# hidasib/GRU4Rec

Measured on AMD Instinct MI355X. Metric: mini-batches/sec (gru4rec.py:661), RSC15-shaped batch=128 n_sample=2048 BPR-max, higher is better.
Workload: dtype f32

## Files before the change

gru4rec_amd/build.py:

```python
import glob
import os
import subprocess
import sys

HERE = os.path.dirname(os.path.abspath(__file__))
SRC = os.path.join(HERE, 'csrc', 'g4r_api.hip')
SRC_HOST = os.path.join(HERE, 'csrc', 'g4r_io.cpp')
OUT = os.path.join(HERE, 'libgru4rec_hip.so')
DEPS = sorted(p for ext in ('hip', 'cuh', 'hpp', 'cpp') for p in glob.glob(os.path.join(HERE, 'csrc', '*.' + ext))) + \
       [os.path.join(os.path.dirname(HERE), 'include', 'gru4rec_hip.h'), os.path.abspath(__file__)]


def build(force=False, verbose=False, out=None, defs=(), flags=()):
    if out is not None:
        return _compile(out, list(defs), verbose, list(flags))
    if not force and os.path.exists(OUT) and all(os.path.getmtime(OUT) >= os.path.getmtime(d) for d in DEPS):
        return OUT
    return _compile(OUT, [], verbose)


COMMON_FLAGS = ['-mllvm', '-amdgpu-kernarg-preload-count=16']


MUTANTS = {1: 'sparse accumulator increments x 1.01', 2: 'sparse Adagrad steps x 1.01', 3: 'dense accumulator increments x 1.01',
# ... 7 lines not shown
           10: "k_replay_final (g4r_recommend_sessions) reads every row's final state from the buffer of the chunk's LONGEST history",
           11: "k_score_cand (g4r_score_candidates*): a work item past a row's first slice reads the items of the row's first slice",
           12: "the two-stage top-k (g4r_recommend_*_scan) ranks its candidates by the APPROXIMATE bf16 scores: the fp32 re-scoring is skipped",
           13: "cosine (g4r_similar_items): the candidate's inverse norm is read at the candidate POSITION instead of its item index",
           14: "k_rollout_feed (g4r_continue_sessions): the sorted insertion drops an item that sorts ABOVE every item already in the row's "
               "exclusion list, so it is never excluded and can be generated again",
           15: "k_beam_advance (g4r_beam_sessions) reads the hidden state of beam row i ITSELF instead of the row of its parent: a new beam "
               "carries on from the wrong state wherever the selection re-parents",
           16: "the owner walk of k_sparse_update_generic drops the first hit of every pass after the first (an item with more than 64 "
               "earlier occurrences in a step loses one of them per later pass)",
           17: "opt_rule's new second statistic (adadelta's update average, Adam's mean) x 1.01",
           18: "k_loss_rows' grp_fast takes a group of V columns whose last column is the first inactive in-batch one (column M) as wholly "
               "active: the unmasked copy of the element loops runs over it",
           19: "k_loss_rows' first pass starts its loop past the prefetched groups one STEP late: the columns of the first trip keep "
               "whatever the LDS held",
           20: "gumbel_noise (g4r_sample_sessions) ignores the decoding step (Philox counter word 2 = 0): every step of a draw gets the "
               "noise of step 0",
           21: "k_owner_window takes the sample-store row of every step of its window from the window's FIRST global step: the owner "
               "tables of the later steps are those of another list",
           22: "hidden_act_bwd decides the branch of leaky / elu / selu on the VALUE of the stored candidate (c >= 0), not on its sign bit: "
               "a pre-activation whose result rounds to -0.0 gets the positive branch's slope",
           23: "hidden_act_bwd: the negative-branch slope of leaky / elu / selu x 1.01",
           24: "k_mmr_rerank (g4r_diversify_*): from the second update on, a position's largest similarity to the picks is OVERWRITTEN by "
               "its similarity to the last pick instead of max-ed with it"}


def mutant_path(k):
    return os.path.join(HERE, '_variants', 'libgru4rec_hip_mut%d.so' % k)


def build_mutants(force=False, verbose=False):
    import fcntl
    from concurrent.futures import ThreadPoolExecutor
    os.makedirs(os.path.join(HERE, '_variants'), exist_ok=True)

    def stale():
        return [k for k in MUTANTS if force or not os.path.exists(mutant_path(k)) or
                any(os.path.getmtime(mutant_path(k)) < os.path.getmtime(d) for d in DEPS)]
    if not stale():
        return [mutant_path(k) for k in MUTANTS]
    with open(os.path.join(HERE, '_variants', '.lock'), 'w') as lock:
        fcntl.flock(lock, fcntl.LOCK_EX)
        todo = stale()
        if todo:
            _host_object(verbose)
            with ThreadPoolExecutor(min(len(todo), 2)) as ex:
                list(ex.map(lambda k: _device(mutant_path(k), ['G4R_MUTATE=%d' % k], verbose, audit=(k != 4)), todo))
# ... 108 lines not shown
```

gru4rec_amd/csrc/g4r_device.cuh:

```cuda
#pragma once
#include <hip/hip_runtime.h>
#include <stdint.h>

#include "../../include/gru4rec_hip.h"

typedef float f32x4 __attribute__((ext_vector_type(4)));

#define G4R_EPS_LOSS 1e-24f
#define G4R_EPS_ADAGRAD 1e-6f
#define G4R_OWN_INLINE 15
#define G4R_OWN_SLOTS 16
#define G4R_OWN_WINDOW_MAXR 12288
#define G4R_OWN_WINDOW_MINWG 4

#if defined(G4R_MUTATE) && G4R_MUTATE == 1
#define G4R_MUT_ACC(x) ((x) * 1.01f)
#else
#define G4R_MUT_ACC(x) (x)
#endif
#if defined(G4R_MUTATE) && G4R_MUTATE == 2
#define G4R_MUT_STEP(x) ((x) * 1.01f)
#else
#define G4R_MUT_STEP(x) (x)
#endif
#if defined(G4R_MUTATE) && G4R_MUTATE == 3
#define G4R_MUT_DACC(x) ((x) * 1.01f)
#else
#define G4R_MUT_DACC(x) (x)
#endif

#if defined(G4R_MUTATE) && G4R_MUTATE == 6
#define G4R_MUT_ROW(n, x) ((n) == 0 ? (x) * 1.5f : (x))
#else
#define G4R_MUT_ROW(n, x) (x)
// ... 13 lines not shown
#else
#define G4R_MUT_PASS_SKIP(pass, ri) false
#endif
#if defined(G4R_MUTATE) && G4R_MUTATE == 17
#define G4R_MUT_STAT2(x) ((x) * 1.01f)
#else
#define G4R_MUT_STAT2(x) (x)
#endif
#if defined(G4R_MUTATE) && G4R_MUTATE == 18
#define G4R_MUT_FAST_M(M) ((M) + 1)
#else
#define G4R_MUT_FAST_M(M) (M)
#endif
#if defined(G4R_MUTATE) && G4R_MUTATE == 19
#define G4R_MUT_FIRST_LATE(step) (step)
#else
#define G4R_MUT_FIRST_LATE(step) 0
#endif

#if defined(G4R_MUTATE) && G4R_MUTATE == 21
#define G4R_MUT_WIN_G(g0, s) (g0)
#else
#define G4R_MUT_WIN_G(g0, s) ((g0) + (s))
#endif

#define G4R_STREAM_SAMPLE 0x53414D50u
#define G4R_STREAM_DROP_EMBED 0x44454D42u
#define G4R_STREAM_DROP_HIDDEN 0x44484944u
#define G4R_STREAM_TIEBREAK 0x54494542u

#if defined(__HIP_DEVICE_COMPILE__)
#define GAS __attribute__((address_space(1)))
#else
#define GAS
#endif
#define GP(T) GAS T*

__device__ __forceinline__ float4 ld4(const GAS float* p) { return *(const GAS float4*)p; }
__device__ __forceinline__ void st4(GAS float* p, float4 v) { *(GAS float4*)p = v; }
__device__ __forceinline__ int4 ldi4(const GAS int* p) { return *(const GAS int4*)p; }
#if defined(__HIP_DEVICE_COMPILE__)
__device__ __forceinline__ float4 ld4(const float* p) { return *(const float4*)p; }
__device__ __forceinline__ void st4(float* p, float4 v) { *(float4*)p = v; }
#endif
__device__ __forceinline__ float4 ld4_if(const GAS float* base, size_t off, bool ok) {
    const float4 v = ld4(base + (ok ? off : (size_t)0));
// ... 263 lines not shown
```

gru4rec_amd/csrc/g4r_host_create.hpp:

```cpp

int g4r_device_count(void) {
    int n = 0;
    if (hipGetDeviceCount(&n) != hipSuccess) return 0;
    return n;
}
const char* g4r_last_error(void) { return g_err.c_str(); }
#ifndef G4R_HIPCC_VERSION
#define G4R_HIPCC_VERSION "unknown"
#endif
const char* g4r_version(void) { return "gru4rec_hip 0.4 (gfx950; hipcc " G4R_HIPCC_VERSION "; isa-audited)"; }
int g4r_sizeof_config(void) { return (int)sizeof(g4r_config); }

static int build_lean_args(g4r_model* m) {
    DevModel& d = m->dm;
    const StepKernels& k = m->kern;
    const int L = d.n_layers;
    std::vector<LeanV> av(L); std::vector<LeanH> ah(L); std::vector<LeanDa> aa(L); std::vector<LeanDy> ay(L);
    const bool constrained = d.embed_mode == G4R_EMBED_CONSTRAINED;
    bool any_layer = false;
    for (int l = 0; l < L; ++l) {
        if (k.fwd[l] != FWD_LEAN) continue;
        any_layer = true;
        LeanV& v = av[l]; memset(&v, 0, sizeof(v));
        v.Wx = d.dense_p + d.offWx[l]; v.Wrz = d.dense_p + d.offWrz[l]; v.Bh = d.dense_p + d.offBh[l];
// ... 33 lines not shown
        q.col_item = d.col_item; q.occ_idx = d.occ_idx + d.B; q.occ_fl = d.occ_fl; q.mp = nullptr; q.dbg = d.dbgclk; q.dbgtile = d.dbgtile; q.R = d.R; q.pub_fl = d.xmode == 0 ? 1 : 0; q.logq = d.logq;
        m->h_leanS = q;
        if (dalloc(m, &m->d_leanS, (size_t)1)) return -1;
    }
    if (k.score_bwd == SB_LEAN) {
        LeanB q; memset(&q, 0, sizeof(q));
        q.accBy = d.accBy; q.occ_fl = d.occ_fl; q.dSy = d.dSy; q.dAy = d.dAy; q.dSBy = d.dSBy; q.dABy = d.dABy; q.dhpart = d.dhpart; q.dbg = d.dbgclk; q.dbgtile = d.dbgtile;
        q.dSy_stride = d.dSy_stride; q.dSBy_stride = d.dSBy_stride; q.defer_mask = d.defer_mask; q.generic = d.generic;
        q.ndh = cdiv(d.Dtop + 1, 64); q.nA = cdiv(d.ldSc, 16) * q.ndh; q.nrb = cdiv(d.B, 16); q.ndb = cdiv(d.Dtop, 64); q.lr = d.lr;
        m->h_leanB = q;
        if (dalloc(m, &m->d_leanB, (size_t)1)) return -1;
        HIPCHK(hipMemcpyAsync(m->d_leanB, &m->h_leanB, sizeof(LeanB), hipMemcpyHostToDevice, m->stream));
    }
    if (k.update == UP_LEAN) {
        LeanU u; memset(&u, 0, sizeof(u));
        u.mp = nullptr; u.st = d.st; u.Wy = d.Wy; u.E = d.E; u.accWy = d.accWy; u.accE = d.accE; u.velWy = d.velWy; u.velE = d.velE;
        u.By = d.By; u.accBy = d.accBy; u.velBy = d.velBy; u.dAx = d.dAx; u.dAy = d.dAy; u.dABy = d.dABy;
        u.dense_p = d.dense_p; u.dense_acc = d.dense_acc; u.dense_vel = d.dense_vel; u.yin0 = d.yin0; u.meta = d.cur_in + 2 * d.B;
        u.dbg = d.dbgclk; u.dbgtile = d.dbgtile; u.n_items = d.n_items; u.constrained = constrained ? 1 : 0; u.wE = d.Ein; u.wY = d.Dtop;
        u.lr = d.lr; u.mom = d.mom; u.lmbd = d.lmbd;
        m->h_leanU = u;
        const std::vector<DenseTile> tiles = dense_tiles(d, 16, 64);
        m->ntiles16 = (int)tiles.size();
        const size_t nslot = cdiv((long long)G4R_OWN_SLOTS * d.R * 16 * sizeof(int), (long long)sizeof(DenseTile));
        if (dalloc(m, &m->d_tiles16, tiles.size() + nslot) || dalloc(m, &m->d_leanU, (size_t)1)) return -1;
        d.own_pos = m->sw.owner_scan_in_update ? nullptr : (int*)(m->d_tiles16 + tiles.size());
        m->h_leanU.own_on = d.own_pos ? 1 : 0;
        const bool pays = cdiv(d.R, LOSS_NW) > G4R_OWN_WINDOW_MINWG;
        m->own_window = d.own_pos && d.R <= G4R_OWN_WINDOW_MAXR && (m->sw.owner_window > 0 || (m->sw.owner_window < 0 && pays));
        HIPCHK(hipMemcpyAsync(m->d_tiles16, tiles.data(), tiles.size() * sizeof(DenseTile), hipMemcpyHostToDevice, m->stream));
        HIPCHK(hipStreamSynchronize(m->stream));
    }
    HIPCHK(hipStreamSynchronize(m->stream));
    return 0;
}

static KernelSwitches read_switches(const g4r_config& cfg) {
    KernelSwitches w;
    w.no_lean = getenv("G4R_NO_LEAN") != nullptr; w.no_mt = getenv("G4R_NO_MT") != nullptr; w.no_bmt = getenv("G4R_NO_BMT") != nullptr;
    w.no_merge = getenv("G4R_NO_MERGE") != nullptr; w.owner_scan_in_update = env_int("G4R_OWNER_SCAN", 0) != 0;
    w.owner_window = env_int("G4R_OWNER_WINDOW", -1);
    w.score_b_split = env_int("G4R_SCORE_B_SPLIT", 1) != 0;
    w.allow_lean_update = env_int("G4R_LEAN_UPDATE", 1) != 0; w.defer = env_int("G4R_DEFER", cfg.defer_updates) != 0;
    w.p2_geo = env_int("G4R_P2_GEO", -1); w.ba_geo = env_int("G4R_BA_GEO", -1);
    w.wide2 = env_int("G4R_WIDE2", -1); w.p1_ks = env_int("G4R_P1_KS", 128); w.bb_ks = env_int("G4R_BB_KS", 0);
    const char* skip = getenv("G4R_SKIP_KN");
    w.skip_kn = skip ? strtoull(skip, nullptr, 0) : 0ull;
    w.trace = getenv("G4R_TRACE") != nullptr;
    return w;
}

int g4r_create(const g4r_config* cfg, g4r_model** out) {
    if (!cfg || !out) return fail("null argument");
    if (cfg->n_layers < 1 || cfg->n_layers > G4R_MAX_LAYERS) return fail("n_layers out of range");
    if (cfg->batch_size < 1 || cfg->n_items < 1) return fail("batch_size / n_items must be positive");
    for (int l = 0; l < cfg->n_layers; ++l)
        if (cfg->layers[l] % 4 != 0 || cfg->layers[l] < 4 || cfg->layers[l] > 1024)
            return fail("layer sizes must be multiples of 4 in [4, 1024]");
    if (cfg->embed_mode == G4R_EMBED_SEPARATE && (cfg->embedding % 4 != 0 || cfg->embedding < 4 || cfg->embedding > 1024))
        return fail("embedding must be a multiple of 4 in [4, 1024]");
    if (cfg->embed_mode != G4R_EMBED_CONSTRAINED && cfg->embed_mode != G4R_EMBED_SEPARATE && cfg->embed_mode != G4R_EMBED_ONEHOT)
        return fail("unsupported embedding mode");
    if (cfg->embed_mode == G4R_EMBED_ONEHOT && 3 * cfg->layers[0] > 1024)
        return fail("one-hot input: 3 * layers[0] must be <= 1024 (row width of the Wx[0] table)");
// ... 225 lines not shown
```

gru4rec_amd/csrc/g4r_host_debug.hpp:

```cpp
int g4r_get_debug(g4r_model* m, const char* name, float* host, int64_t count) {
    if (!m || !name || !host) return fail("null argument");
    HIPCHK(hipSetDevice(m->cfg.device));
    DevModel& d = m->dm;
    const StepKernels& k = m->kern;
    std::string s(name);
    const float* p = nullptr; int64_t n = 0;
    int l = 0;
    if (!s.empty() && isdigit((unsigned char)s.back())) { l = s.back() - '0'; s.pop_back(); }
    if (l >= d.n_layers) return fail("layer out of range");
    const int64_t bd = (int64_t)d.B * d.D[l];
    if (s == "scores") { p = d.Sc; n = (int64_t)d.B * d.ldSc; }
    else if (s == "dSx") { p = d.dSx + (size_t)((m->gstep - 1) & d.defer_mask) * (size_t)d.dSx_stride; n = (int64_t)d.B * d.Ein; }
    else if (s == "dSy") { p = d.dSy + (size_t)((m->gstep - 1) & d.defer_mask) * (size_t)d.dSy_stride; n = (int64_t)d.ldSc * d.Dtop; }
    else if (s == "dSBy") { p = d.dSBy + (size_t)((m->gstep - 1) & d.defer_mask) * (size_t)d.dSBy_stride; n = d.ldSc; }
    else if (s == "defer_stats") {
        if (count < 4) return fail("count");
        double rows = 0, bias = 0;
        if (m->defer_on) {
            std::vector<unsigned> st(2048);
            HIPCHK(hipStreamSynchronize(m->stream));
            HIPCHK(hipMemcpy(st.data(), d.dstat, st.size() * sizeof(unsigned), hipMemcpyDeviceToHost));
            for (size_t i = 0; i < st.size(); i += 2) { rows += st[i]; bias += st[i + 1]; }
        }
        host[0] = (float)rows; host[1] = (float)bias; host[2] = m->defer_on ? 1.f : 0.f; host[3] = (float)(d.defer_mask + 1);
// ... 15 lines not shown
        host[0] = (float)m->ro_calls; host[1] = (float)m->ro_steps;
        return 0;
    }
    else if (s == "events_launches") {
        if (count < 4) return fail("count");
        host[0] = (float)m->ev_steps; host[1] = (float)m->ev_scans; host[2] = (float)m->ev_launches; host[3] = (float)m->ev_pieces;
        return 0;
    }
    else if (s == "dhpart") { p = d.dhpart; n = (int64_t)d.ksplit * d.B * d.Dtop; }
    else if (s == "lossrow") { p = d.lossrow; n = d.B; }
    else if (s == "hd") { p = d.hd[l]; n = bd; }
    else if (s == "r") { p = d.r[l]; n = bd; }
    else if (s == "z") { p = d.z[l]; n = bd; }
    else if (s == "c") { p = d.c[l]; n = bd; }
    else if (s == "Hr") { p = d.Hr[l]; n = bd; }
    else if (s == "dV") { p = d.dV[l]; n = bd * 3; }
    else if (s == "dyl") { p = d.dyl[l]; n = bd; }
    else if (s == "Hprev") { p = d.H[l][(m->gstep + 1) & 1]; n = bd; }
    else if (s == "occ_idx") { p = (const float*)d.occ_idx; n = d.R; }
    else if (s == "own_pos") {
        if (!d.own_pos) return fail("no owner table (k_update_l not chosen, or G4R_OWNER_SCAN=1)");
        p = (const float*)(d.own_pos + (m->own_window ? (size_t)m->own_last * d.R * 16 : (size_t)0)); n = 16 * (int64_t)d.R;
    }
    else if (s == "own_pos_ring") { if (!d.own_pos) return fail("no owner table (k_update_l not chosen, or G4R_OWNER_SCAN=1)"); p = (const float*)d.own_pos; n = (int64_t)G4R_OWN_SLOTS * 16 * d.R; }
    else if (s == "owner_window") { if (count < 1) return fail("count"); host[0] = (m->own_window && k.update == UP_LEAN) ? 1.f : 0.f; return 0; }
#if !defined(G4R_CLK_TRACE)
    else if (s == "dbgclk" || s == "dbgtile") return fail("in-kernel traces need a library built with G4R_BUILD_CLK=1 (python -m gru4rec_amd.build --force) and G4R_CLK=1 at run time");
#endif
    else if (s == "dbgclk") { if (!d.dbgclk) return fail("G4R_CLK not set"); p = (const float*)d.dbgclk; n = 2 * (64 + 8 * (int64_t)d.R); }
    else if (s == "dbgtile") { if (!d.dbgtile) return fail("G4R_CLK not set"); p = (const float*)d.dbgtile; n = 2 * 8 * (int64_t)8192; }
    else if (s == "ntiles") { if (count < 1) return fail("count"); host[0] = (float)m->ntiles; return 0; }
    else if (s == "ldSc") { if (count < 1) return fail("count"); host[0] = (float)d.ldSc; return 0; }
    else if (s == "wide_mask") {
        if (count < 1) return fail("count");
        int mk = k.wide_dense ? 16 : 0;
        for (int l = 0; l < d.n_layers; ++l) mk |= k.wg[l].use;
        host[0] = (float)mk; return 0;
    }
    else if (s == "deep_geo") {
        if (count < 1) return fail("count");
        host[0] = (float)(k.p2_deep[0] + 2 * k.ba_deep[0]); return 0;
    }
    else if (s == "score_mt") { if (count < 1) return fail("count"); host[0] = k.score_fwd == SF_MT ? 272.f : 0.f; return 0; }
    else if (s == "score_bmt") { if (count < 1) return fail("count"); host[0] = (float)k.bmt_slabs; return 0; }
    else if (s == "lean") {
        if (count < 4) return fail("count");
        int mk = 0;
// ... 208 lines not shown
```

gru4rec_amd/csrc/g4r_host_model.hpp:

```cpp
static thread_local std::string g_err;
static int fail(const std::string& s) { g_err = s; return -1; }
void g4r_set_error(const char* fmt, ...) {
    char buf[1024];
    va_list ap;
    va_start(ap, fmt);
    vsnprintf(buf, sizeof(buf), fmt, ap);
    va_end(ap);
    g_err = buf;
}
#define HIPCHK(x)                                                                                        \
    do {                                                                                                 \
        hipError_t e_ = (x);                                                                             \
        if (e_ != hipSuccess)                                                                            \
            return fail(std::string(#x) + ": " + hipGetErrorString(e_) + " @" + std::to_string(__LINE__)); \
    } while (0)
#define NCCLCHK(x)                                                                                         \
    do {                                                                                                   \
        ncclResult_t e_ = (x);                                                                             \
        if (e_ != ncclSuccess)                                                                             \
            return fail(std::string(#x) + ": " + ncclGetErrorString(e_) + " @" + std::to_string(__LINE__)); \
    } while (0)

enum { KN_GRU_P1 = 0, KN_GRU_P2, KN_SCORE_FWD, KN_LOSS, KN_SCORE_BWD, KN_BWD_PRE, KN_BWD_A, KN_BWD_B, KN_DENSE, KN_ALLREDUCE,
       KN_DENSE_APPLY, KN_SPARSE, KN_UPDATE, KN_BWD_FUSED, KN_FWD_FUSED, KN_GATE, KN_FLUSH, KN_SCAN, KN_FINISH, KN_GRU_V, KN_GRU_H, KN_GRU_DA, KN_GRU_DY, KN_OWNER_WINDOW, KN_COUNT };
static const char* KN_NAMES[KN_COUNT] = {"k_gru_p1", "k_gru_p2", "k_score_fwd", "k_loss_rows", "k_score_bwd", "k_gru_bwd_pre",
                                         "k_gru_bwd_a", "k_gru_bwd_b", "k_dense_grad", "rccl_allreduce", "k_dense_apply",
                                         "k_sparse_update", "k_update", "k_gru_bwd", "k_gru_fwd", "k_gru_gate", "k_sparse_flush", "k_defer_scan", "k_finish_rows", "k_gru_v", "k_gru_h", "k_gru_da", "k_gru_dy", "k_owner_window"};

struct EvRec { int kn; hipEvent_t a, b; };

struct KernelSwitches {
    bool no_lean = false;
    bool no_mt = false, no_bmt = false;
    bool no_merge = false;
    bool allow_lean_update = true;
    bool score_b_split = true;
    bool owner_scan_in_update = false;
    int owner_window = -1;
    bool defer = false;
    int p2_geo = -1, ba_geo = -1;
    int wide2 = -1, p1_ks = 128, bb_ks = 0;
    unsigned long long skip_kn = 0;
    bool trace = false;
};
enum GruFwdKind { FWD_LEAN = 0 , FWD_FUSED = 1 , FWD_P1S = 2 ,
                  FWD_P1_N64 = 3, FWD_P1_N32 = 4 };
enum GruBwdKind { BWD_LEAN = 0 , BWD_FUSED = 1 , BWD_ONEHOT = 2, BWD_BW = 3, BWD_B = 4 };
enum ScoreFwdKind { SF_LEAN = 0 , SF_MT = 1 , SF_T3 = 2, SF_T2 = 3, SF_K64 = 4, SF_K128 = 5  };
enum ScoreBwdKind { SB_LEAN = 0 , SB_BMT = 1 , SB_BWD2 = 2 , SB_W = 3, SB_N = 4  };
enum UpdateKind { UP_LEAN = 0 , UP_MERGED = 1 , UP_SPLIT = 2 };
struct WideGeo { int use = 0, ny = 1, nh = 1, kys = 0, khs = 0, bbn = 1, bbk = 0; };
struct StepKernels {
    int fwd[G4R_MAX_LAYERS], bwd[G4R_MAX_LAYERS];
    int p2_deep[G4R_MAX_LAYERS], ba_deep[G4R_MAX_LAYERS];
    WideGeo wg[G4R_MAX_LAYERS];
    int score_fwd;
    int loss_spec, loss_long, loss_quads;
    int score_bwd;
    int score_a_host;
    int kch, ksplit;
    int bmt_slabs;
// ... 33 lines not shown
    int64_t gstep = 0;
    DenseTile* d_tiles = nullptr;
    int ntiles = 0, nblk_occ = 0, nblk_occ_g = 0;
    size_t smem_score = 0, smem_loss = 0, smem_sparse = 0;
    bool defer_on = false;
    bool defer_broken = false;
    hipEvent_t ev_df[4] = {nullptr, nullptr, nullptr, nullptr};
    DenseTile* d_tiles64 = nullptr;
    int ntiles64 = 0;
    float* d_tmpH = nullptr;
    LeanS h_leanS;
    std::vector<LeanV> h_leanV; std::vector<LeanH> h_leanH; std::vector<LeanDa> h_leanDa; std::vector<LeanDy> h_leanDy;
    LeanS* d_leanS = nullptr;
    LeanB* d_leanB = nullptr; LeanB h_leanB;
    LeanU* d_leanU = nullptr; LeanU h_leanU;
    DenseTile* d_tiles16 = nullptr; int ntiles16 = 0;
    bool own_window = false;
    int own_last = 0;
    hipEvent_t ev_ow[2] = {nullptr, nullptr};
    LeanV* d_leanV = nullptr; LeanH* d_leanH = nullptr; LeanDa* d_leanDa = nullptr; LeanDy* d_leanDy = nullptr;
    hipGraphExec_t gexec = nullptr;
    hipGraphExec_t gexec_small = nullptr;
    hipGraphExec_t gexec_head = nullptr;
    int graph_steps = 0;
    bool dist_graph_failed = false;
    bool profiling = false;
    bool profile_split = false;
    bool exact = false;
    size_t smem_exact = 0;
    double kn_ms[KN_COUNT] = {0};
    int64_t kn_n[KN_COUNT] = {0};
    std::vector<hipEvent_t> evs;
    int pbatch = 0, ppar = 0;
    float* pH[G4R_MAX_LAYERS][2] = {{nullptr}};
    float* phout[G4R_MAX_LAYERS] = {nullptr};
    float *pVc[G4R_MAX_LAYERS] = {nullptr}, *pz[G4R_MAX_LAYERS] = {nullptr}, *pHr[G4R_MAX_LAYERS] = {nullptr};
    int *p_in = nullptr, *p_tgt = nullptr, *p_keep = nullptr;
    DevBuf<int> p_items;
    unsigned char* p_zero = nullptr;
    float* p_ranks = nullptr;
    DevBuf<float> p_scores;
    int* p_cnt = nullptr;
    int64_t p_nsel = 0, p_ldo = 0;
    DevBuf<uint2> p_topk;
    DevBuf<int> p_tcols;
    DevBuf<float> p_tscores;
    DevBuf<long long> p_xoffs;
// ... 51 lines not shown
    std::vector<SyncPlane> planes[2];
    int sync_rule[2] = {G4R_SYNC_MEAN, G4R_SYNC_SUM};
    bool sync_rule_user = false;
    unsigned char* d_touched = nullptr;
    unsigned char* d_rowcnt = nullptr;
    int sync_every_dev = 0;
    int64_t since_sync = 0, n_dev_syncs = 0;
    struct Scratch { void* p = nullptr; size_t cap = 0; bool host = false; };
    Scratch sc_ids, sc_blk, sc_cnt, sc_all, sc_send, sc_pack, sc_recv, sc_hall;
    float* d_dense[2] = {nullptr, nullptr};
    bool sync_on = false;
};

struct MmrStage {
    int tab; const float* T; int W;
    bool cosine;
    float lam; int normalize;
    int k;
    int32_t* out_pos; float* out_value;
};

static inline void weights_changed(g4r_model* m) { m->s_tab_valid = false; m->sim_valid[0] = m->sim_valid[1] = false; }
static inline void drop_step_graphs(g4r_model* m, bool also_head) {
    for (hipGraphExec_t* g : {&m->gexec, &m->gexec_small, also_head ? &m->gexec_head : nullptr})
        if (g && *g) { (void)hipGraphExecDestroy(*g); *g = nullptr; }
}

enum StepMode { STEP_GRAPH, STEP_HEAD_GRAPH, STEP_EAGER };
static inline bool local_staged(const g4r_model* m) {
    return !m->dm.apply_dense_inplace && m->cfg.nranks <= 1 && !m->comm_ready && !m->p2p_ready && !m->virtual_ranks;
}
static inline bool dist_graph_wanted(const g4r_model* m) {
    return !m->dm.apply_dense_inplace && !m->dist_graph_failed && (m->p2p_ready || m->comm_ready || local_staged(m));
}
static inline StepMode step_mode(const g4r_model* m) {
    if (!m->cfg.use_graph || m->profiling || m->sw.trace) return STEP_EAGER;
    return (m->dm.apply_dense_inplace || dist_graph_wanted(m)) ? STEP_GRAPH : STEP_HEAD_GRAPH;
}
static inline StepMode single_step_mode(const g4r_model* m, StepMode mode) {
    if (mode != STEP_GRAPH) return mode;
    return m->dm.apply_dense_inplace ? STEP_EAGER : STEP_HEAD_GRAPH;
}

template <class T>
static int dalloc(g4r_model* m, T** p, size_t n, bool zero = true) {
    void* q = nullptr;
    if (n == 0) n = 1;
    HIPCHK(hipMalloc(&q, n * sizeof(T)));
// ... 61 lines not shown
static const size_t SMEM_P1 = tile_smem<GT_BM, GT_BN, P1_BK, false, false>() + GT_BM * sizeof(int);
static constexpr auto k_gru_p2_w4 = k_gru_p2<GT_NTH, GT_BK>;
static constexpr auto k_gru_p2_w8d = k_gru_p2<512, 256>;
static const size_t SMEM_P2_256 = tile_smem<GT_BM, GT_BN, 256, false, false>() + GT_BM * sizeof(int);
static constexpr auto k_gru_bwd_a_w4 = k_gru_bwd_a<GT_NTH, GT_BK>;
static constexpr auto k_gru_bwd_a_w8d = k_gru_bwd_a<512, 256>;
static const size_t SMEM_BA_256 = tile_smem<GT_BM, GT_BN, 256, false, true>();
static const size_t SMEM_BB = tile_smem<GT_BM, GT_BN, BB_BK, false, true>() + GT_BM * sizeof(int);
static constexpr auto k_score_fwd_k128 = k_score_fwd<GT_BN, GT_BK>;
#define SFW_BN 32
#define SFW_BK 64
static constexpr auto k_score_fwd_k64 = k_score_fwd<SFW_BN, SFW_BK>;
static constexpr auto k_score_fwd_t2 = k_score_fwd<64, 32, T2_BK>;
static const size_t SMEM_SF2 = (size_t)Tile2Cfg<T2_BK>::SMEM_FLOATS * sizeof(float);
static constexpr auto k_score_fwd_t3 = k_score_fwd<64, 32, 3>;
static const size_t SMEM_SF3 = (size_t)Tile3Cfg<T3_NST, T3_BKS>::SMEM_FLOATS * sizeof(float);
static const size_t SMEM_BMT = std::max((size_t)BMT_NST_A * BMT_STAGE_A * sizeof(float), (size_t)BMT_NST_B * BMT_STAGE_B * sizeof(float) + 2048 * sizeof(int));
static const size_t SMEM_SF64 = tile_smem<SF_BM, SFW_BN, SFW_BK, false, true>() + SFW_BN * sizeof(int);
static constexpr auto k_score_bwd_n = k_score_bwd<32, GT_BK>;
static constexpr auto k_score_bwd_w = k_score_bwd<64, 64>;
static const size_t SMEM_SBW = std::max(tile_smem<64, 64, 64, true, false>(), tile_smem<64, 64, 64, false, false>());
#define ZROW_FLOATS 8192
#define G4R_DEFER_SLOTS 16
static_assert(G4R_OWN_SLOTS == G4R_DEFER_SLOTS, "the windows of g4r_train_steps serve the deferral ring and the owner ring alike");
static const size_t SMEM_SF = tile_smem<SF_BM, GT_BN, GT_BK, false, true>() + GT_BN * sizeof(int);
static constexpr auto k_score_mt_4s = k_score_mt<4, true>;
static const size_t SMEM_MT_4S = (size_t)MtCfg<4, true>::SMEM_FLOATS * sizeof(float);
static const size_t SMEM_T2K = (size_t)(4 * 64 * 16) * sizeof(float);
static const size_t SMEM_T3 = (size_t)Tile3Cfg<3, 32>::SMEM_FLOATS * sizeof(float);

static constexpr decltype(&k_loss_rows<false, 0, 1>) K_LOSS_ROWS[3][4] = {
    {k_loss_rows<false, 0, 1>, k_loss_rows<false, 1, 1>, k_loss_rows<false, 2, 1>, k_loss_rows<false, 3, 1>},
    {k_loss_rows<false, 0, 4>, k_loss_rows<false, 1, 4>, k_loss_rows<false, 2, 4>, k_loss_rows<false, 3, 4>},
    {k_loss_rows<true, 0, 4>, k_loss_rows<true, 1, 4>, k_loss_rows<true, 2, 4>, k_loss_rows<true, 3, 4>}};
static inline auto loss_rows_kernel(const StepKernels& k) { return K_LOSS_ROWS[k.loss_long ? 2 : (k.loss_quads ? 1 : 0)][k.loss_spec]; }
static inline int chunk_index(int chunks) { return chunks == 1 ? 0 : (chunks == 2 ? 1 : 2); }
static constexpr decltype(&k_sparse_update<1, false>) K_SPARSE_UPDATE[3][2] = {
    {k_sparse_update<1, false>, k_sparse_update<1, true>}, {k_sparse_update<2, false>, k_sparse_update<2, true>}, {k_sparse_update<4, false>, k_sparse_update<4, true>}};
static constexpr decltype(&k_sparse_update_generic<1>) K_SPARSE_UPDATE_GENERIC[3] = {k_sparse_update_generic<1>, k_sparse_update_generic<2>, k_sparse_update_generic<4>};
static constexpr decltype(&k_update<1, 32, false>) K_UPDATE[2][2] = {{k_update<1, 32, false>, k_update<1, 32, true>}, {k_update<2, 32, false>, k_update<2, 32, true>}};

static std::vector<DenseTile> dense_tiles(const DevModel& d, int TR, int TC) {
    std::vector<DenseTile> tiles;
    for (int l = 0; l < d.n_layers; ++l) {
        const int D = d.D[l], IN = d.IN[l];
        auto add = [&](const float* x0, const float* x1, int ldx, int nrows, int ncols, int coff, int ldo, long long base) {
            for (int r = 0; r < nrows; r += TR)
// ... 115 lines not shown
```

gru4rec_amd/csrc/g4r_host_step.hpp:

```cpp
extern "C++" {
struct StepLauncher {
    g4r_model* m;
    hipStream_t s;
    std::vector<EvRec>* recs;
    size_t evi = 0;
    int kn = -1;
    hipEvent_t ev_a = nullptr, ev_b = nullptr;
    StepLauncher(g4r_model* m_, std::vector<EvRec>* recs_) : m(m_), s(m_->stream), recs(recs_) {}
    void use(int kn_, hipEvent_t a, hipEvent_t b) { kn = kn_; ev_a = a; ev_b = b; }
    void open(int kn_) {
        if (m->sw.trace) { fprintf(stderr, "[g4r] launch %s\n", KN_NAMES[kn_]); fflush(stderr); }
        use(kn_, nullptr, nullptr);
        if (!recs) return;
        while (m->evs.size() < evi + 2) { hipEvent_t e; (void)hipEventCreate(&e); m->evs.push_back(e); }
        use(kn_, m->evs[evi], m->evs[evi + 1]);
        evi += 2;
        recs->push_back(EvRec{kn_, ev_a, ev_b});
    }
    bool skipped() const { return m->sw.skip_kn && kn >= 0 && ((m->sw.skip_kn >> kn) & 1ull); }
    template <class... P, class... A>
    void launch(void (*kern)(P...), dim3 grid, dim3 block, size_t smem, A... a) {
        if (skipped()) return;
        if (ev_a) hipExtLaunchKernelGGL(kern, grid, block, (unsigned)smem, s, ev_a, ev_b, 0, static_cast<P>(a)...);
        else hipLaunchKernelGGL(kern, grid, block, smem, s, static_cast<P>(a)...);
// ... 312 lines not shown
    e = hipGraphInstantiate(out, graph, nullptr, nullptr, 0);
    (void)hipGraphDestroy(graph);
    if (e != hipSuccess) { *out = nullptr; (void)hipGetLastError(); return fail(std::string("graph instantiate: ") + hipGetErrorString(e)); }
    return 0;
}
static int ensure_graph(g4r_model* m) {
    if (m->gexec) return 0;
    const bool dist = !m->dm.apply_dense_inplace && !local_staged(m);
    const bool rccl_in_graph = dist && (!m->p2p_ready || (m->exact && m->comm_ready));
    if (dist) {
        if (!m->p2p_ready) NCCLCHK(ncclAllReduce(m->dm.dense_g, m->dm.dense_g, m->dm.dense_count, ncclFloat, ncclSum, m->comm, m->stream));
        if (m->exact && m->comm_ready)
            NCCLCHK(ncclAllGather((const float*)m->dm.xbase + (size_t)m->cfg.rank * (size_t)m->dm.xstride, (float*)m->dm.xbase, (size_t)m->dm.xstride,
                                  ncclFloat, m->comm, m->stream));
        HIPCHK(hipStreamSynchronize(m->stream));
    }
    if (capture_steps(m, G4R_GRAPH_STEPS, rccl_in_graph ? hipStreamCaptureModeRelaxed : hipStreamCaptureModeThreadLocal, &m->gexec)) return -1;
    m->graph_steps = G4R_GRAPH_STEPS;
    if (!dist) {
        if (capture_steps(m, G4R_GRAPH_STEPS_SMALL, hipStreamCaptureModeThreadLocal, &m->gexec_small)) m->gexec_small = nullptr;
    }
    return 0;
}
static int ensure_head_graph(g4r_model* m) {
    if (m->gexec_head) return 0;
    hipGraph_t graph;
    StepLauncher lk(m, nullptr);
    HIPCHK(hipStreamBeginCapture(m->stream, hipStreamCaptureModeThreadLocal));
    if (step_head(m, lk, 0)) { hipGraph_t g2; (void)hipStreamEndCapture(m->stream, &g2); return -1; }
    HIPCHK(hipStreamEndCapture(m->stream, &graph));
    HIPCHK(hipGraphInstantiate(&m->gexec_head, graph, nullptr, nullptr, 0));
    (void)hipGraphDestroy(graph);
    return 0;
}
static int ensure_step_graph(g4r_model* m) {
    if (m->dm.apply_dense_inplace) return ensure_graph(m);
    if (dist_graph_wanted(m)) {
        if (ensure_graph(m) == 0) return 0;
        m->dist_graph_failed = true;
        fprintf(stderr, "[g4r] RCCL all-reduce could not be captured into the step graph (%s); launching it eagerly\n", g_err.c_str());
    }
    return ensure_head_graph(m);
}

struct StepWindow {
    g4r_model* m;
    const bool own_win;
    bool scanned = false;
    explicit StepWindow(g4r_model* m_) : m(m_), own_win(m_->own_window && m_->kern.update == UP_LEAN && !(m_->profiling && m_->profile_split)) {}
    ~StepWindow() { if (scanned) m->defer_broken = true; }
    bool on() const { return m->defer_on || own_win; }
    int open(int64_t t, int64_t g, int64_t nw) {
        const DevModel& d = m->dm;
        const DevModel* dmp = (const DevModel*)m->d_dm;
        if (own_win) {
            StepLauncher lk(m, nullptr);
            if (m->profiling) for (auto& e : m->ev_ow) if (!e) (void)hipEventCreate(&e);
            lk.use(KN_OWNER_WINDOW, m->profiling ? m->ev_ow[0] : nullptr, m->profiling ? m->ev_ow[1] : nullptr);
            lk.launch(k_owner_window, dim3((unsigned)(nw * cdiv(2 * d.B, OW_NW))), dim3(OW_T), (size_t)(((d.R + 3) & ~3) + 16 * OW_NW) * sizeof(int), dmp, t, g, nw);
            HIPCHK(hipGetLastError());
        }
        if (!m->defer_on) return 0;
        scanned = true;
        const dim3 gs(cdiv(nw * d.R, 256));
        if (m->profiling) (void)hipEventRecord(m->ev_df[0], m->stream);
        hipLaunchKernelGGL(k_defer_scan, gs, dim3(256), 0, m->stream, dmp, (long long)t, (long long)g, (int)nw, 0);
        hipLaunchKernelGGL(k_defer_scan, gs, dim3(256), 0, m->stream, dmp, (long long)t, (long long)g, (int)nw, 1);
        if (m->profiling) (void)hipEventRecord(m->ev_df[1], m->stream);
        return 0;
    }
    int close(int64_t g, int64_t nw) {
        auto timed = [&](int kn, hipEvent_t a, hipEvent_t b) {
            float ms = 0.f;
            if (hipEventElapsedTime(&ms, a, b) == hipSuccess) { m->kn_ms[kn] += ms; m->kn_n[kn]++; }
        };
        if (own_win) {
            m->own_last = (int)nw - 1;
            if (m->profiling) {
                HIPCHK(hipStreamSynchronize(m->stream));
                timed(KN_OWNER_WINDOW, m->ev_ow[0], m->ev_ow[1]);
            }
        }
// ... 47 lines not shown
    if (mode == STEP_GRAPH && !m->dm.apply_dense_inplace) {
        if (ensure_step_graph(m)) return -1;
        mode = step_mode(m);
    }
    const StepMode single = single_step_mode(m, mode);
    size_t ci = std::lower_bound(m->compact_steps.begin(), m->compact_steps.end(), t0) - m->compact_steps.begin();
    int64_t t = t0;
    const int64_t tend = t0 + n_steps;
    std::vector<EvRec> recs;
    while (t < tend) {
        if (between_steps(m, t, &ci)) return -1;
        const bool devsync = m->sync_every_dev > 0 && m->comm_ready;
        if (devsync && m->since_sync >= m->sync_every_dev) {
            if (sync_dense_enqueue(m)) return -1;
            ++m->n_dev_syncs;
        }
        int64_t run = tend - t;
        if (devsync) run = std::min<int64_t>(run, m->sync_every_dev - m->since_sync);
        if (ci < m->compact_steps.size()) run = std::min(run, m->compact_steps[ci] - t);
        if (m->dm.ns > 0 && !m->store_frozen) run = std::min<int64_t>(run, m->gl - (m->gstep % m->gl));
        if (run <= 0) return fail("internal: empty run");
        const bool replay = mode == STEP_GRAPH && run >= G4R_GRAPH_STEPS_SMALL;
        if (replay && ensure_graph(m)) return -1;
        for (int64_t done = 0, nw; done < run; done += nw) {
            const int64_t left = run - done;
            hipGraphExec_t g = nullptr;
            if (replay && left >= m->graph_steps) { g = m->gexec; nw = m->graph_steps; }
            else if (replay && m->gexec_small && left >= G4R_GRAPH_STEPS_SMALL) { g = m->gexec_small; nw = G4R_GRAPH_STEPS_SMALL; }
            else nw = win.on() ? std::min<int64_t>(G4R_DEFER_SLOTS, left) : 1;
            const bool windowed = g || win.on();
            if (windowed && win.open(t + done, m->gstep + done, nw)) return -1;
            if (g) HIPCHK(hipGraphLaunch(g, m->stream));
            else for (int i = 0; i < nw; ++i) if (single_step(m, single, windowed ? i : 0, recs)) return -1;
            if (windowed && win.close(m->gstep + done, nw)) return -1;
        }
        t += run;
        m->gstep += run;
        m->since_sync += run;
    }
    HIPCHK(hipStreamSynchronize(m->stream));
    if (m->p2p_ready) {
        unsigned late = 0;
        HIPCHK(hipMemcpy(&late, m->p2p_round + m->p2p_nblk, sizeof(late), hipMemcpyDeviceToHost));
        if (late) return fail("p2p all-reduce: a peer did not publish its gradients within G4R_P2P_TIMEOUT_MS (dead rank?)");
    }
    return 0;
}

int g4r_virtual_train_steps(g4r_model* const* ms, int32_t n, int64_t t0, int64_t n_steps) {
    if (!ms || n < 1 || n > 16) return fail("virtual ranks: 1..16 handles");
// ... 114 lines not shown
```

gru4rec_amd/csrc/g4r_update_kernels.cuh:

```cuda
#pragma once
__global__ __launch_bounds__(256) void k_onehot_step(const DevModel* __restrict__ mp, StepState* st) {
    const DevModel& m = *mp;
    const StepCtx c = load_ctx(st);
    const int W = m.Ein, nc4 = W >> 2;
    const long long q = (long long)blockIdx.x * 256 + threadIdx.x;
    const int row = (int)(q / nc4), c4 = (int)(q % nc4);
    if (row >= c.M) return;
    const int item = m.occ_idx[row];
    if (item < 0) return;
    const float lr = m.lr;
    const float4 g = ld4(m.dV[0] + (size_t)row * W + 4 * c4);
    const float4 a = ld4(m.accE + (size_t)item * W + 4 * c4);
    const int cnt = m.occ_fl[4 * ((size_t)m.n_items + item) + 2];
    const float4 an = make_float4(a.x + g.x * g.x, a.y + g.y * g.y, a.z + g.z * g.z, a.w + g.w * g.w);
    if (!m.generic && cnt == 1) st4(m.accE + (size_t)item * W + 4 * c4, an);
    else st4(m.dAx + (size_t)row * W + 4 * c4, an);
    if (m.generic) { st4(G4R_DSX(m, c.g) + (size_t)row * W + 4 * c4, g); return; }
    st4(G4R_DSX(m, c.g) + (size_t)row * W + 4 * c4, make_float4(lr * g.x * frsq(an.x + G4R_EPS_ADAGRAD), lr * g.y * frsq(an.y + G4R_EPS_ADAGRAD),
                                                         lr * g.z * frsq(an.z + G4R_EPS_ADAGRAD), lr * g.w * frsq(an.w + G4R_EPS_ADAGRAD)));
}

struct DenseTile {
    GP(const float) X0; GP(const float) X1; GP(const float) dV;
    long long base;
// ... 496 lines not shown
    const int B = m.B, M = m.Mplan[t];
    table = 0;
    int item = -1;
    if (k < B) { if (k < M) item = m.in_idx[t * B + k]; table = (m.embed_mode == G4R_EMBED_CONSTRAINED) ? 0 : 1; }
    else if (k < 2 * B) { if (k - B < M) item = m.out_idx[t * B + (k - B)]; }
    else if (M > 0) item = m.ST[(size_t)(m.gl > 0 ? g % m.gl : 0) * m.ns + (k - 2 * B)];
    return item;
}
__global__ __launch_bounds__(256) void k_defer_scan(const DevModel* __restrict__ mp, long long t0, long long g0, int n, int pass) {
    const DevModel& m = *mp;
    const long long idx = (long long)blockIdx.x * 256 + threadIdx.x;
    const int R = m.R, s = (int)(idx / R), k = (int)(idx - (long long)s * R);
    if (s >= n) return;
    int table;
    const int item = defer_item(m, t0 + s, g0 + s, k, table);
    const size_t slot = G4R_SLOT(m, g0 + s) * (size_t)m.dRcap + k;
    if (item < 0) { if (pass) m.dcand[slot] = 0; return; }
    GAS int* lu = m.last_use + (size_t)table * m.n_items + item;
    if (pass == 0) atomicMax((int*)lu, (int)(g0 + s));
    else m.dcand[slot] = (*lu == (int)(g0 + s)) ? 1 : 0;
}
#define OW_T 1024
#define OW_NW (OW_T / 64)
static_assert(G4R_OWN_INLINE + 1 == 16, "an owner-table row is 16 ints: the count and G4R_OWN_INLINE positions");
static_assert(((size_t)G4R_OWN_WINDOW_MAXR + 16 * OW_NW) * sizeof(int) <= 65536, "k_owner_window: the longest list and the waves' position rows share one workgroup's 64 KB of LDS");
__global__ __launch_bounds__(OW_T) void k_owner_window(const DevModel* __restrict__ mp, long long t0, long long g0, int nw) {
    const DevModel& m = *mp;
    extern __shared__ __attribute__((aligned(16))) int sid[];
    const int R = m.R, B = m.B, Rp = (R + 3) & ~3;
    const int gps = (2 * B + OW_NW - 1) / OW_NW;
    const int s = (int)blockIdx.x / gps, q = (int)blockIdx.x - s * gps;
#if defined(G4R_CLK_TRACE)
    struct Span { GAS long long* p; __device__ ~Span() { if (p) p[1] = wall_clock64(); } } span_{(m.dbgtile && threadIdx.x == 0 && blockIdx.x < 400) ? m.dbgtile + 8 * (size_t)(7700 + blockIdx.x) : nullptr};
    if (span_.p) span_.p[0] = wall_clock64();
#endif
    if (s >= nw) return;
    for (int k = threadIdx.x; k < Rp; k += OW_T) {
        int table;
        sid[k] = k < R ? defer_item(m, t0 + s, G4R_MUT_WIN_G(g0, s), k, table) : -1;
    }
    __syncthreads();
    const int lane = threadIdx.x & 63, wid = threadIdx.x >> 6;
    const int p = q * OW_NW + wid;
    if (p >= 2 * B) return;
    const int item = sid[p];
    if (item < 0) return;
    const bool constrained = m.embed_mode == G4R_EMBED_CONSTRAINED;
    const int ta = (constrained || p < B) ? 0 : B, tb = (!constrained && p < B) ? B : R;
    int* spos = sid + Rp + 16 * wid;
    const unsigned long long below = (1ull << lane) - 1ull;
    int cnt = 0, last = p;
    for (int base0 = ta & ~3; base0 < tb; base0 += 1024) {
        int4 vv[4];
#pragma unroll
        for (int u = 0; u < 4; ++u) vv[u] = *(const int4*)(sid + min(base0 + 256 * u + 4 * lane, Rp - 4));
#pragma unroll
        for (int u = 0; u < 4; ++u) {
            const int j0 = base0 + 256 * u + 4 * lane;
            const int ids[4] = {vv[u].x, vv[u].y, vv[u].z, vv[u].w};
            bool hit[4], anyl = false;
#pragma unroll
            for (int e = 0; e < 4; ++e) { hit[e] = ids[e] == item && j0 + e >= ta && j0 + e < tb; anyl = anyl || hit[e]; }
            if (__ballot(anyl) == 0ull) continue;
            unsigned long long mk[4];
            int at = cnt;
#pragma unroll
            for (int e = 0; e < 4; ++e) {
                mk[e] = __ballot(hit[e]);
                at += __popcll(mk[e] & below);
            }
            const unsigned long long any = mk[0] | mk[1] | mk[2] | mk[3];
            if (cnt == 0) {
                const int l0 = __builtin_ctzll(any);
                int e0 = 3;
#pragma unroll
                for (int e = 2; e >= 0; --e) if ((mk[e] >> l0) & 1ull) e0 = e;
                if (base0 + 256 * u + 4 * l0 + e0 != p) return;
            }
            const int lh = 63 - __builtin_clzll(any);
#pragma unroll
            for (int e = 0; e < 4; ++e) if ((mk[e] >> lh) & 1ull) last = base0 + 256 * u + 4 * lh + e;
#pragma unroll
            for (int e = 0; e < 4; ++e) {
                if (hit[e]) {
                    if (at <= G4R_OWN_INLINE) spos[at] = j0 + e;
                    ++at;
                }
                cnt += __popcll(mk[e]);
            }
        }
    }
    if (cnt < 2) return;
    GAS int* pos = m.own_pos + ((size_t)s * (size_t)R + (size_t)last) * 16;
    if (cnt - 1 > G4R_OWN_INLINE) {
        if (lane == 0) pos[0] = -1;
        return;
    }
    __builtin_amdgcn_fence(__ATOMIC_ACQ_REL, "wavefront");
    if (lane < cnt - 1) pos[1 + lane] = spos[lane];
    if (lane == 0) pos[0] = cnt - 1;
}
#define FL_NR 4
__global__ __launch_bounds__(SP_WAVES * 64) void k_sparse_flush(const DevModel* __restrict__ mp, long long g0, int n) {
    const DevModel& m = *mp;
    const int lane = threadIdx.x & 63, wid = threadIdx.x >> 6;
    const long long e0 = ((long long)blockIdx.x * SP_WAVES + wid) * FL_NR;
    const int Rc = m.dRcap, s = (int)(e0 / Rc), k0 = (int)(e0 - (long long)s * Rc);
    if (s >= n) return;
    const size_t slot = G4R_SLOT(m, g0 + s) * (size_t)Rc + k0;
    int it[FL_NR];
#pragma unroll
    for (int u = 0; u < FL_NR; ++u) it[u] = m.dlist[slot + u];
    if (lane < FL_NR) { m.dcand[slot + lane] = 0; m.dlist[slot + lane] = -1; }
    const int B = m.B;
    const bool sep = m.embed_mode != G4R_EMBED_CONSTRAINED;
    const GAS float *sx = G4R_DSX(m, g0 + s), *sy = G4R_DSY(m, g0 + s), *sb = G4R_DSBY(m, g0 + s);
// ... 383 lines not shown
```

Before: 26940.

## Add long graph windows backed by a larger owner ring, batch owner-window id loads

Enlarges the owner-position ring from 16 to up to 128 slots, capped by a byte budget, and captures an additional long HIP graph (32 steps by default) so that each graph launch and each k_owner_window launch covers more training steps. The owner-window kernel now loads the step's item ids directly in unrolled batches of four with hoisted scalar arguments, instead of calling defer_item once per element. The aim is to cut per-window launch and graph-replay overhead and to speed up the id-fill prologue. In exchange it uses more device memory, adds one more graph capture, and adds a configuration check that can reject invalid G4R_GRAPH_STEPS_LONG values.

```diff
diff --git a/gru4rec_amd/build.py b/gru4rec_amd/build.py
--- a/gru4rec_amd/build.py
+++ b/gru4rec_amd/build.py
@@ -53,7 +53,9 @@
                "a pre-activation whose result rounds to -0.0 gets the positive branch's slope",
            23: "hidden_act_bwd: the negative-branch slope of leaky / elu / selu x 1.01",
            24: "k_mmr_rerank (g4r_diversify_*): from the second update on, a position's largest similarity to the picks is OVERWRITTEN by "
-               "its similarity to the last pick instead of max-ed with it"}
+               "its similarity to the last pick instead of max-ed with it",
+           25: "k_owner_window writes the owner table of step s of its window into slot s & 15 of the ring: past the 16th step of a long "
+               "window the tables land on those of the first 16 steps"}
 
 
 def mutant_path(k):
diff --git a/gru4rec_amd/csrc/g4r_device.cuh b/gru4rec_amd/csrc/g4r_device.cuh
--- a/gru4rec_amd/csrc/g4r_device.cuh
+++ b/gru4rec_amd/csrc/g4r_device.cuh
@@ -9,7 +9,8 @@
 #define G4R_EPS_LOSS 1e-24f
 #define G4R_EPS_ADAGRAD 1e-6f
 #define G4R_OWN_INLINE 15
-#define G4R_OWN_SLOTS 16
+#define G4R_OWN_SLOTS 128
+#define G4R_OWN_RING_MAXBYTES (32u << 20)
 #define G4R_OWN_WINDOW_MAXR 12288
 #define G4R_OWN_WINDOW_MINWG 4
 
@@ -69,6 +70,11 @@
 #define G4R_MUT_WIN_G(g0, s) (g0)
 #else
 #define G4R_MUT_WIN_G(g0, s) ((g0) + (s))
+#endif
+#if defined(G4R_MUTATE) && G4R_MUTATE == 25
+#define G4R_MUT_WIN_SLOT(s) ((s) & 15)
+#else
+#define G4R_MUT_WIN_SLOT(s) (s)
 #endif
 
 #define G4R_STREAM_SAMPLE 0x53414D50u
diff --git a/gru4rec_amd/csrc/g4r_host_create.hpp b/gru4rec_amd/csrc/g4r_host_create.hpp
--- a/gru4rec_amd/csrc/g4r_host_create.hpp
+++ b/gru4rec_amd/csrc/g4r_host_create.hpp
@@ -79,12 +79,18 @@
         m->h_leanU = u;
         const std::vector<DenseTile> tiles = dense_tiles(d, 16, 64);
         m->ntiles16 = (int)tiles.size();
-        const size_t nslot = cdiv((long long)G4R_OWN_SLOTS * d.R * 16 * sizeof(int), (long long)sizeof(DenseTile));
+        const bool pays = cdiv(d.R, LOSS_NW) > G4R_OWN_WINDOW_MINWG;
+        m->own_window = !m->sw.owner_scan_in_update && d.R <= G4R_OWN_WINDOW_MAXR && (m->sw.owner_window > 0 || (m->sw.owner_window < 0 && pays));
+        int nlong = m->sw.graph_steps_long;
+        if (nlong < 0 || nlong > G4R_OWN_SLOTS || (nlong & (nlong - 1))) return fail("G4R_GRAPH_STEPS_LONG: 0, or a power of two from 16 to 128");
+        if (!(m->own_window && d.apply_dense_inplace && !m->defer_on)) nlong = 0;
+        while (nlong > 16 && (size_t)nlong * d.R * 16 * sizeof(int) > (size_t)G4R_OWN_RING_MAXBYTES) nlong /= 2;
+        m->graph_steps_long = nlong > 16 ? nlong : 0;
+        m->own_slots = std::max(16, m->graph_steps_long);
+        const size_t nslot = cdiv((long long)m->own_slots * d.R * 16 * sizeof(int), (long long)sizeof(DenseTile));
         if (dalloc(m, &m->d_tiles16, tiles.size() + nslot) || dalloc(m, &m->d_leanU, (size_t)1)) return -1;
         d.own_pos = m->sw.owner_scan_in_update ? nullptr : (int*)(m->d_tiles16 + tiles.size());
         m->h_leanU.own_on = d.own_pos ? 1 : 0;
-        const bool pays = cdiv(d.R, LOSS_NW) > G4R_OWN_WINDOW_MINWG;
-        m->own_window = d.own_pos && d.R <= G4R_OWN_WINDOW_MAXR && (m->sw.owner_window > 0 || (m->sw.owner_window < 0 && pays));
         HIPCHK(hipMemcpyAsync(m->d_tiles16, tiles.data(), tiles.size() * sizeof(DenseTile), hipMemcpyHostToDevice, m->stream));
         HIPCHK(hipStreamSynchronize(m->stream));
     }
@@ -96,7 +102,7 @@
     KernelSwitches w;
     w.no_lean = getenv("G4R_NO_LEAN") != nullptr; w.no_mt = getenv("G4R_NO_MT") != nullptr; w.no_bmt = getenv("G4R_NO_BMT") != nullptr;
     w.no_merge = getenv("G4R_NO_MERGE") != nullptr; w.owner_scan_in_update = env_int("G4R_OWNER_SCAN", 0) != 0;
-    w.owner_window = env_int("G4R_OWNER_WINDOW", -1);
+    w.owner_window = env_int("G4R_OWNER_WINDOW", -1); w.graph_steps_long = env_int("G4R_GRAPH_STEPS_LONG", G4R_GRAPH_STEPS_LONG);
     w.score_b_split = env_int("G4R_SCORE_B_SPLIT", 1) != 0;
     w.allow_lean_update = env_int("G4R_LEAN_UPDATE", 1) != 0; w.defer = env_int("G4R_DEFER", cfg.defer_updates) != 0;
     w.p2_geo = env_int("G4R_P2_GEO", -1); w.ba_geo = env_int("G4R_BA_GEO", -1);
diff --git a/gru4rec_amd/csrc/g4r_host_debug.hpp b/gru4rec_amd/csrc/g4r_host_debug.hpp
--- a/gru4rec_amd/csrc/g4r_host_debug.hpp
+++ b/gru4rec_amd/csrc/g4r_host_debug.hpp
@@ -61,7 +61,13 @@
         if (!d.own_pos) return fail("no owner table (k_update_l not chosen, or G4R_OWNER_SCAN=1)");
         p = (const float*)(d.own_pos + (m->own_window ? (size_t)m->own_last * d.R * 16 : (size_t)0)); n = 16 * (int64_t)d.R;
     }
-    else if (s == "own_pos_ring") { if (!d.own_pos) return fail("no owner table (k_update_l not chosen, or G4R_OWNER_SCAN=1)"); p = (const float*)d.own_pos; n = (int64_t)G4R_OWN_SLOTS * 16 * d.R; }
+    else if (s == "own_pos_ring") {
+        if (!d.own_pos) return fail("no owner table (k_update_l not chosen, or G4R_OWNER_SCAN=1)");
+        const int64_t tab = 16 * (int64_t)d.R;
+        if (count < tab || count % tab || count / tab > m->own_slots) return fail("own_pos_ring: a whole number of tables of 16 R ints, from 1 to the ring's " + std::to_string(m->own_slots));
+        p = (const float*)d.own_pos; n = count;
+    }
+    else if (s == "graph_steps_long") { if (count < 1) return fail("count"); host[0] = (float)long_window_steps(m); return 0; }
     else if (s == "owner_window") { if (count < 1) return fail("count"); host[0] = (m->own_window && k.update == UP_LEAN) ? 1.f : 0.f; return 0; }
 #if !defined(G4R_CLK_TRACE)
     else if (s == "dbgclk" || s == "dbgtile") return fail("in-kernel traces need a library built with G4R_BUILD_CLK=1 (python -m gru4rec_amd.build --force) and G4R_CLK=1 at run time");
diff --git a/gru4rec_amd/csrc/g4r_host_model.hpp b/gru4rec_amd/csrc/g4r_host_model.hpp
--- a/gru4rec_amd/csrc/g4r_host_model.hpp
+++ b/gru4rec_amd/csrc/g4r_host_model.hpp
@@ -29,6 +29,8 @@
 
 struct EvRec { int kn; hipEvent_t a, b; };
 
+#define G4R_GRAPH_STEPS_LONG 32
+static_assert(G4R_GRAPH_STEPS_LONG <= G4R_OWN_SLOTS && (G4R_GRAPH_STEPS_LONG & (G4R_GRAPH_STEPS_LONG - 1)) == 0, "the long window: a power of two the owner ring can hold");
 struct KernelSwitches {
     bool no_lean = false;
     bool no_mt = false, no_bmt = false;
@@ -37,6 +39,7 @@
     bool score_b_split = true;
     bool owner_scan_in_update = false;
     int owner_window = -1;
+    int graph_steps_long = G4R_GRAPH_STEPS_LONG;
     bool defer = false;
     int p2_geo = -1, ba_geo = -1;
     int wide2 = -1, p1_ks = 128, bb_ks = 0;
@@ -116,7 +119,10 @@
     hipGraphExec_t gexec = nullptr;
     hipGraphExec_t gexec_small = nullptr;
     hipGraphExec_t gexec_head = nullptr;
+    hipGraphExec_t gexec_long = nullptr;
     int graph_steps = 0;
+    int graph_steps_long = 0;
+    int own_slots = 16;
     bool dist_graph_failed = false;
     bool profiling = false;
     bool profile_split = false;
@@ -214,8 +220,11 @@
 
 static inline void weights_changed(g4r_model* m) { m->s_tab_valid = false; m->sim_valid[0] = m->sim_valid[1] = false; }
 static inline void drop_step_graphs(g4r_model* m, bool also_head) {
-    for (hipGraphExec_t* g : {&m->gexec, &m->gexec_small, also_head ? &m->gexec_head : nullptr})
+    for (hipGraphExec_t* g : {&m->gexec, &m->gexec_small, &m->gexec_long, also_head ? &m->gexec_head : nullptr})
         if (g && *g) { (void)hipGraphExecDestroy(*g); *g = nullptr; }
+}
+static inline int long_window_steps(const g4r_model* m) {
+    return (m->own_window && m->kern.update == UP_LEAN && m->dm.apply_dense_inplace && !m->defer_on) ? m->graph_steps_long : 0;
 }
 
 enum StepMode { STEP_GRAPH, STEP_HEAD_GRAPH, STEP_EAGER };
@@ -323,7 +332,7 @@
 static const size_t SMEM_SBW = std::max(tile_smem<64, 64, 64, true, false>(), tile_smem<64, 64, 64, false, false>());
 #define ZROW_FLOATS 8192
 #define G4R_DEFER_SLOTS 16
-static_assert(G4R_OWN_SLOTS == G4R_DEFER_SLOTS, "the windows of g4r_train_steps serve the deferral ring and the owner ring alike");
+static_assert(G4R_OWN_SLOTS >= G4R_DEFER_SLOTS, "the windows of g4r_train_steps serve the deferral ring and the owner ring alike; only the owner ring has long windows");
 static const size_t SMEM_SF = tile_smem<SF_BM, GT_BN, GT_BK, false, true>() + GT_BN * sizeof(int);
 static constexpr auto k_score_mt_4s = k_score_mt<4, true>;
 static const size_t SMEM_MT_4S = (size_t)MtCfg<4, true>::SMEM_FLOATS * sizeof(float);
diff --git a/gru4rec_amd/csrc/g4r_host_step.hpp b/gru4rec_amd/csrc/g4r_host_step.hpp
--- a/gru4rec_amd/csrc/g4r_host_step.hpp
+++ b/gru4rec_amd/csrc/g4r_host_step.hpp
@@ -358,6 +358,12 @@
     }
     return 0;
 }
+static int ensure_long_graph(g4r_model* m, int n) {
+    if (m->gexec_long) return 0;
+    if (capture_steps(m, n, hipStreamCaptureModeThreadLocal, &m->gexec_long)) return -1;
+    (void)hipGraphUpload(m->gexec_long, m->stream);
+    return 0;
+}
 static int ensure_head_graph(g4r_model* m) {
     if (m->gexec_head) return 0;
     hipGraph_t graph;
@@ -390,10 +396,11 @@
         const DevModel& d = m->dm;
         const DevModel* dmp = (const DevModel*)m->d_dm;
         if (own_win) {
+            if (nw > m->own_slots) return fail("internal: a window longer than the owner ring");
             StepLauncher lk(m, nullptr);
             if (m->profiling) for (auto& e : m->ev_ow) if (!e) (void)hipEventCreate(&e);
             lk.use(KN_OWNER_WINDOW, m->profiling ? m->ev_ow[0] : nullptr, m->profiling ? m->ev_ow[1] : nullptr);
-            lk.launch(k_owner_window, dim3((unsigned)(nw * cdiv(2 * d.B, OW_NW))), dim3(OW_T), (size_t)(((d.R + 3) & ~3) + 16 * OW_NW) * sizeof(int), dmp, t, g, nw);
+            lk.launch(k_owner_window, dim3((unsigned)(nw * cdiv(2 * d.B, OW_NW))), dim3(OW_T), OW_SMEM(d.R), dmp, t, g, nw);
             HIPCHK(hipGetLastError());
         }
         if (!m->defer_on) return 0;
@@ -487,10 +494,13 @@
         if (run <= 0) return fail("internal: empty run");
         const bool replay = mode == STEP_GRAPH && run >= G4R_GRAPH_STEPS_SMALL;
         if (replay && ensure_graph(m)) return -1;
+        const int64_t nlong = replay ? long_window_steps(m) : 0;
+        if (nlong && run >= nlong && ensure_long_graph(m, (int)nlong)) return -1;
         for (int64_t done = 0, nw; done < run; done += nw) {
             const int64_t left = run - done;
             hipGraphExec_t g = nullptr;
-            if (replay && left >= m->graph_steps) { g = m->gexec; nw = m->graph_steps; }
+            if (nlong && left >= nlong) { g = m->gexec_long; nw = nlong; }
+            else if (replay && left >= m->graph_steps) { g = m->gexec; nw = m->graph_steps; }
             else if (replay && m->gexec_small && left >= G4R_GRAPH_STEPS_SMALL) { g = m->gexec_small; nw = G4R_GRAPH_STEPS_SMALL; }
             else nw = win.on() ? std::min<int64_t>(G4R_DEFER_SLOTS, left) : 1;
             const bool windowed = g || win.on();
diff --git a/gru4rec_amd/csrc/g4r_update_kernels.cuh b/gru4rec_amd/csrc/g4r_update_kernels.cuh
--- a/gru4rec_amd/csrc/g4r_update_kernels.cuh
+++ b/gru4rec_amd/csrc/g4r_update_kernels.cuh
@@ -542,12 +542,25 @@
 }
 #define OW_T 1024
 #define OW_NW (OW_T / 64)
+#define OW_U 4
+#define OW_IDS(R) (((R) + OW_U * OW_T - 1) / (OW_U * OW_T) * (OW_U * OW_T))
+#define OW_SMEM(R) ((size_t)(OW_IDS(R) + 16 * OW_NW) * sizeof(int))
 static_assert(G4R_OWN_INLINE + 1 == 16, "an owner-table row is 16 ints: the count and G4R_OWN_INLINE positions");
-static_assert(((size_t)G4R_OWN_WINDOW_MAXR + 16 * OW_NW) * sizeof(int) <= 65536, "k_owner_window: the longest list and the waves' position rows share one workgroup's 64 KB of LDS");
+static_assert(OW_SMEM(G4R_OWN_WINDOW_MAXR) <= 65536, "k_owner_window: the longest list and the waves' position rows share one workgroup's 64 KB of LDS");
 __global__ __launch_bounds__(OW_T) void k_owner_window(const DevModel* __restrict__ mp, long long t0, long long g0, int nw) {
     const DevModel& m = *mp;
     extern __shared__ __attribute__((aligned(16))) int sid[];
-    const int R = m.R, B = m.B, Rp = (R + 3) & ~3;
+    const int R = m.R, B = m.B, Rp = (R + 3) & ~3, Rs = OW_IDS(R), ns = m.ns, gl = m.gl;
+    const int emode = m.embed_mode;
+    const GAS int* const Mplan = m.Mplan;
+    const GAS int* const in_idx = m.in_idx;
+    const GAS int* const out_idx = m.out_idx;
+    const GAS int* const ST = m.ST;
+    GAS int* const own_pos = m.own_pos;
+#if defined(__HIP_DEVICE_COMPILE__)
+    asm volatile("" ::"s"(R), "s"(B), "s"(ns), "s"(gl), "s"(emode), "s"(Mplan), "s"(in_idx), "s"(out_idx), "s"(ST), "s"(own_pos));
+#endif
+    const bool constrained = emode == G4R_EMBED_CONSTRAINED;
     const int gps = (2 * B + OW_NW - 1) / OW_NW;
     const int s = (int)blockIdx.x / gps, q = (int)blockIdx.x - s * gps;
 #if defined(G4R_CLK_TRACE)
@@ -555,9 +568,29 @@
     if (span_.p) span_.p[0] = wall_clock64();
 #endif
     if (s >= nw) return;
-    for (int k = threadIdx.x; k < Rp; k += OW_T) {
-        int table;
-        sid[k] = k < R ? defer_item(m, t0 + s, G4R_MUT_WIN_G(g0, s), k, table) : -1;
+    {
+        const long long t = t0 + s;
+        const int M = Mplan[t];
+        const GAS int* xin = in_idx + t * B;
+        const GAS int* yout = out_idx + t * B;
+        const GAS int* srow = ST + (size_t)(gl > 0 ? G4R_MUT_WIN_G(g0, s) % gl : 0) * ns;
+#pragma clang loop unroll(disable) vectorize(disable) interleave(disable)
+        for (int k0 = threadIdx.x; k0 < Rs; k0 += OW_U * OW_T) {
+            int v[OW_U];
+#pragma unroll
+            for (int u = 0; u < OW_U; ++u) {
+                const int kc = min(k0 + u * OW_T, R - 1);
+                const bool isx = kc < B, isy = kc < 2 * B;
+                const GAS int* base = isx ? xin : (isy ? yout : srow);
+                v[u] = base[kc - (isx ? 0 : (isy ? B : 2 * B))];
+            }
+#pragma unroll
+            for (int u = 0; u < OW_U; ++u) {
+                const int k = k0 + u * OW_T;
+                const int row = k < B ? k : (k < 2 * B ? k - B : 0);
+                sid[k] = (k < R && row < M) ? v[u] : -1;
+            }
+        }
     }
     __syncthreads();
     const int lane = threadIdx.x & 63, wid = threadIdx.x >> 6;
@@ -565,9 +598,8 @@
     if (p >= 2 * B) return;
     const int item = sid[p];
     if (item < 0) return;
-    const bool constrained = m.embed_mode == G4R_EMBED_CONSTRAINED;
     const int ta = (constrained || p < B) ? 0 : B, tb = (!constrained && p < B) ? B : R;
-    int* spos = sid + Rp + 16 * wid;
+    int* spos = sid + Rs + 16 * wid;
     const unsigned long long below = (1ull << lane) - 1ull;
     int cnt = 0, last = p;
     for (int base0 = ta & ~3; base0 < tb; base0 += 1024) {
@@ -611,7 +643,7 @@
         }
     }
     if (cnt < 2) return;
-    GAS int* pos = m.own_pos + ((size_t)s * (size_t)R + (size_t)last) * 16;
+    GAS int* pos = own_pos + ((size_t)G4R_MUT_WIN_SLOT(s) * (size_t)R + (size_t)last) * 16;
     if (cnt - 1 > G4R_OWN_INLINE) {
         if (lane == 0) pos[0] = -1;
         return;
```

Result: slower. 25510 (-5.3%).
